# dongyunjinyu/YOLO-Lite

Hardware: NVIDIA B200
Metric: images_per_sec (higher is better)
Workload: dtype bf16

## Files before the change

include/yl11.h:

```cpp
#ifndef YL11_H
#define YL11_H

#include <stddef.h>
#include <stdint.h>

#ifdef __cplusplus
extern "C" {
#endif

#define YL11_VERSION 200

typedef enum yl_status {
    YL_OK = 0,
    YL_ERR_ARG = -1,
    YL_ERR_CUDA = -2,
    YL_ERR_UNSUPPORTED = -3,
    YL_ERR_WORKSPACE = -4,
    YL_ERR_NO_DEVICE = -5
} yl_status;

typedef enum yl_dtype { YL_BF16 = 0, YL_F32 = 1, YL_U8 = 2, YL_F16 = 3 } yl_dtype;
typedef enum yl_act { YL_ACT_NONE = 0, YL_ACT_SILU = 1 } yl_act;
typedef enum yl_conv_impl { YL_IMPL_AUTO = 0, YL_IMPL_DIRECT = 1, YL_IMPL_TCGEN05 = 2 } yl_conv_impl;

// ... 86 lines not shown
int yl_dw_pw_det_supported(const yl_conv_args* pw, const yl_conv_args* head);
int yl_dw_pw_det(const yl_conv_args* pw, const void* dw_w, const float* dw_bias, int dw_act, const yl_conv_args* head, void* stream);

int yl_sppf_pool(const yl_tensor* x, const yl_tensor* y1, const yl_tensor* y2, const yl_tensor* y3, int k,
                 void* stream);

int yl_psa_attention(const yl_tensor* qkv, const yl_tensor* out, int heads, int key_dim, int head_dim,
                     float scale, void* stream);

int yl_detect_decode(const yl_tensor* levels, int nl, const float* strides_host, int reg_max, int nc, float* y,
                     void* stream);

int yl_dfl(const float* x, float* y, int b, int reg_max, int a, void* stream);

size_t yl_nms_workspace_bytes(int B, int A, int nc, int multi_label);
int yl_nms_batched(const float* pred, int B, int nc, int A, float conf_thres, double iou_thres,
                   const int32_t* classes_dev, int n_classes, int agnostic, int multi_label, int max_det,
                   int max_nms, float max_wh, void* workspace, size_t workspace_bytes, float* out,
                   int32_t* counts, void* stream);
int yl_nms_begin(void* workspace, size_t workspace_bytes, int B, void* stream);
int yl_debug_nms_phases(long long* device_buf);
int yl_nms_select(const float* pred, int B, int nc, int A, double iou_thres, int agnostic, int max_det, int max_nms,
                  float max_wh, void* workspace, size_t workspace_bytes, float* out, int32_t* counts, void* stream);
size_t yl_nms_boxes_workspace_bytes(int n);
int yl_nms_boxes(const float* boxes, const float* scores, int n, double iou_thres, void* workspace,
                 size_t workspace_bytes, int64_t* keep, int32_t* count, void* stream);
int yl_xywh2xyxy_inplace(float* pred, int B, int C, int A, void* stream);
int yl_scale_boxes(float* dets, const int32_t* counts, int B, int max_det, const float* params_dev, void* stream);

int yl_to_f32(const void* x, int x_dtype, float* y, long long n, void* stream);

int yl_stem_fused_supported(int ci, int c0, int c1);
int yl_stem_fused(const void* x_nchw, int x_dtype, int n, int ci, int h, int w, const void* w0, int ci_pad0,
                  const float* b0, int act0, const void* w1, int ci_pad1, const float* b1, int act1, const yl_tensor* y,
                  void* stream);

int yl_c3k2_tail_supported(int c, int c2);
int yl_c3k2_tail(const yl_tensor* t, const yl_tensor* y, const void* wa, const float* ba, int wa_co_pad, int wa_ci_pad,
                 const void* wb, const float* bb, int wb_ci_pad, const void* w2, const float* b2, int w2_ci_pad,
                 int shortcut, void* stream);
int yl_c3k2_tail_tc(const yl_tensor* t, const yl_tensor* y, const void* wa, const float* ba, int wa_co_pad, int wa_ci_pad,
                 const void* wb, const float* bb, int wb_ci_pad, const void* w2, const float* b2, int w2_ci_pad,
                 int shortcut, void* stream);

int yl_match_predictions(const float* dets, const int32_t* counts, int B, int max_det, const float* gt_boxes,
                         const float* gt_cls, const int32_t* gt_offsets, int max_labels_per_image,
                         const float* iou_thresholds_dev, int n_thresholds, uint8_t* tp, void* stream);

typedef struct yl_lb_image {
    const uint8_t* src;
    int32_t sh, sw, pitch;
    int32_t new_w, new_h, left, top;
    int32_t _pad;
} yl_lb_image;
int yl_letterbox_u8(const yl_lb_image* imgs_dev, int n, float* dst_nchw, int H, int W, int pad_value, void* stream);

typedef struct yl_tta_canvas {
    float* y;
    int32_t H, W;
    int32_t h, w;
    int32_t flip;
    int32_t _pad;
} yl_tta_canvas;
int yl_tta_scale_img(const void* x, int x_dtype, int n, int c, int h, int w, const yl_tta_canvas* canvases, void* stream);
typedef struct yl_tta_pass {
    const float* pred;
    int32_t A;
    int32_t a0, n;
// ... 11 lines not shown
```

yolo-lite_b200/csrc/stem_fused.cu:

```cuda
#include <cuda_fp16.h>

#include "common.cuh"

namespace yl {

struct StemFusedParams {
    const void* x;
    int N, CI, H, W;
    const __nv_bfloat16* w0;
    int ci_pad0;
    const float* b0;
    const __nv_bfloat16* w1;
    const float* b1;
    __nv_bfloat16* y;
    long long y_cstride;
    int y_coff;
    int H0, W0, H1, W1;
    int act0, act1;
    int tiles_w, tiles_h, total_tiles;
};

__device__ __forceinline__ void sf_ldsm_x4(uint32_t addr, uint32_t& r0, uint32_t& r1, uint32_t& r2, uint32_t& r3) {
    asm volatile("ldmatrix.sync.aligned.m8n8.x4.shared.b16 {%0,%1,%2,%3}, [%4];"
                 : "=r"(r0), "=r"(r1), "=r"(r2), "=r"(r3)
                 : "r"(addr));
}
__device__ __forceinline__ void sf_mma(float (&d)[4], const uint32_t (&a)[4], uint32_t b0, uint32_t b1) {
    asm volatile(
        "mma.sync.aligned.m16n8k16.row.col.f32.bf16.bf16.f32 {%0,%1,%2,%3}, {%4,%5,%6,%7}, {%8,%9}, {%0,%1,%2,%3};"
        : "+f"(d[0]), "+f"(d[1]), "+f"(d[2]), "+f"(d[3])
        : "r"(a[0]), "r"(a[1]), "r"(a[2]), "r"(a[3]), "r"(b0), "r"(b1));
}

template <typename T> struct SfQuad;
template <> struct SfQuad<float> {
    using raw = float4;
    static __device__ __forceinline__ raw zero() { return make_float4(0.f, 0.f, 0.f, 0.f); }
    static __device__ __forceinline__ raw load(const float* p) { return __ldg(reinterpret_cast<const float4*>(p)); }
    static __device__ __forceinline__ float4 widen(raw v) { return v; }
    static __device__ __forceinline__ float one(const float* p) { return __ldg(p); }
};
template <> struct SfQuad<__half> {
    using raw = uint2;
    static __device__ __forceinline__ raw zero() { return make_uint2(0u, 0u); }
    static __device__ __forceinline__ raw load(const __half* p) { return __ldg(reinterpret_cast<const uint2*>(p)); }
    static __device__ __forceinline__ float4 widen(raw v) {
        const float2 a = __half22float2(*reinterpret_cast<const __half2*>(&v.x));
        const float2 b = __half22float2(*reinterpret_cast<const __half2*>(&v.y));
        return make_float4(a.x, a.y, b.x, b.y);
    }
    static __device__ __forceinline__ float one(const __half* p) { return __half2float(*p); }
};
template <> struct SfQuad<uint8_t> {
    using raw = uint32_t;
    static __device__ __forceinline__ raw zero() { return 0u; }
    static __device__ __forceinline__ raw load(const uint8_t* p) { return __ldg(reinterpret_cast<const uint32_t*>(p)); }
    static __device__ __forceinline__ float4 widen(raw v) {
        return make_float4(__fdiv_rn((float)(v & 0xffu), 255.f), __fdiv_rn((float)((v >> 8) & 0xffu), 255.f),
                           __fdiv_rn((float)((v >> 16) & 0xffu), 255.f), __fdiv_rn((float)(v >> 24), 255.f));
    }
    static __device__ __forceinline__ float one(const uint8_t* p) { return __fdiv_rn((float)__ldg(p), 255.f); }
};

constexpr int SF_TH = 8, SF_TW = 16;
constexpr int SF_R0 = 2 * SF_TH + 1, SF_C0 = 2 * SF_TW + 1;
constexpr int SF_RI = 2 * SF_R0 + 1;
constexpr int SF_CI = 72;
constexpr int SF_M0 = (SF_R0 * SF_C0 + 15) / 16;
constexpr int SF_EC = (SF_C0 + 1) / 2;
constexpr int SF_P0 = 48;
constexpr int SF_W1S = 9 * 16 * 2 + 16;
constexpr int SF_OFF_IN = 0;
constexpr int SF_OFF_L0 = SF_OFF_IN + SF_RI * SF_CI * 8;
constexpr int SF_OFF_W1 = SF_OFF_L0 + 2 * SF_R0 * SF_EC * SF_P0;
constexpr int SF_OFF_B = SF_OFF_W1 + 32 * SF_W1S;
constexpr int SF_OFF_TAB = SF_OFF_B + 48 * 4;
constexpr int SF_SMEM = SF_OFF_TAB + SF_M0 * 16 * 8;

template <typename TIn>
__global__ void __launch_bounds__(256, 2) stem_fused_kernel(const StemFusedParams p) {
    using Q = SfQuad<TIn>;
    const TIn* px_in = reinterpret_cast<const TIn*>(p.x);
    extern __shared__ __align__(16) uint8_t sf_smem[];
    griddep_launch_dependents();
    const int lane = threadIdx.x & 31, warp = threadIdx.x >> 5;
    const int g = lane >> 2, t = lane & 3;
    uint2* s_in = reinterpret_cast<uint2*>(sf_smem + SF_OFF_IN);
    const uint32_t sL0 = smem_u32(sf_smem + SF_OFF_L0), sW1 = smem_u32(sf_smem + SF_OFF_W1);
    float* sb0 = reinterpret_cast<float*>(sf_smem + SF_OFF_B);
    float* sb1 = sb0 + 16;

    for (int i = threadIdx.x; i < 32 * (SF_W1S / 16); i += blockDim.x) {
        const int r = i / (SF_W1S / 16), u = i - r * (SF_W1S / 16);
        uint4 v = make_uint4(0u, 0u, 0u, 0u);
        if (u < 18) v = __ldg(reinterpret_cast<const uint4*>(p.w1 + (size_t)r * 144) + u);
        *reinterpret_cast<uint4*>(sf_smem + SF_OFF_W1 + r * SF_W1S + u * 16) = v;
    }
    if (threadIdx.x < 16) sb0[threadIdx.x] = __ldg(p.b0 + threadIdx.x);
    if (threadIdx.x < 32) sb1[threadIdx.x] = __ldg(p.b1 + threadIdx.x);
    uint32_t bw0[3][2][2];
#pragma unroll
    for (int nt = 0; nt < 2; ++nt) {
        const __nv_bfloat16* wrow = p.w0 + (size_t)(nt * 8 + g) * 9 * p.ci_pad0;
#pragma unroll
        for (int ks = 0; ks < 3; ++ks)
#pragma unroll
            for (int hh = 0; hh < 2; ++hh) {
                uint32_t v = 0;
#pragma unroll
                for (int e = 0; e < 2; ++e) {
                    const int k = 16 * ks + 2 * t + e + hh * 8;
                    const int tap = k >> 2, ci = k & 3;
                    uint32_t bits = 0;
                    if (tap < 9 && ci < p.CI) bits = (uint32_t)__bfloat16_as_ushort(wrow[tap * p.ci_pad0 + ci]);
                    v |= bits << (16 * e);
                }
                bw0[ks][nt][hh] = v;
            }
    }
    int woff[3][2];
#pragma unroll
    for (int ks = 0; ks < 3; ++ks)
#pragma unroll
        for (int hh = 0; hh < 2; ++hh) {
            const int k = 16 * ks + 2 * t + hh * 8;
            const int tap = k >> 2, r = tap / 3, s2 = tap - 3 * r;
            woff[ks][hh] = tap < 9 ? ((r * SF_CI + s2) * 2 + ((k >> 1) & 1)) : 0;
        }
    uint2* s_tab = reinterpret_cast<uint2*>(sf_smem + SF_OFF_TAB);
    for (int i = threadIdx.x; i < SF_M0 * 16; i += blockDim.x) {
        const bool valid = i < SF_R0 * SF_C0;
        const int idx = valid ? i : SF_R0 * SF_C0 - 1;
// ... 133 lines not shown

        {
            const int r = warp;
            const int lrow = lane & 15, khalf = lane >> 4;
            float acc[4][4];
#pragma unroll
            for (int nt = 0; nt < 4; ++nt) {
                const float2 bb = *reinterpret_cast<const float2*>(sb1 + nt * 8 + 2 * t);
                acc[nt][0] = bb.x; acc[nt][1] = bb.y; acc[nt][2] = bb.x; acc[nt][3] = bb.y;
            }
            const uint32_t brow = sW1 + (uint32_t)(((lane >> 4) * 8 + (lane & 7)) * SF_W1S + 8 * ((lane >> 3) & 1) * 2);
#pragma unroll
            for (int t3 = 0; t3 < 9; t3 += 3) {
                uint32_t a[3][4], b[3][2][4];
#pragma unroll
                for (int j = 0; j < 3; ++j) {
                    const int tap = t3 + j, dr = tap / 3, dc = tap - 3 * dr;
                    const uint32_t arow = sL0 + (uint32_t)((((dc & 1) * SF_R0 + 2 * r + dr) * SF_EC + lrow + (dc >> 1)) * SF_P0 +
                                                           khalf * 16);
                    sf_ldsm_x4(arow, a[j][0], a[j][1], a[j][2], a[j][3]);
#pragma unroll
                    for (int np = 0; np < 2; ++np)
                        sf_ldsm_x4(brow + (uint32_t)(np * 16 * SF_W1S + tap * 32), b[j][np][0], b[j][np][1], b[j][np][2],
                                   b[j][np][3]);
                }
#pragma unroll
                for (int j = 0; j < 3; ++j)
#pragma unroll
                    for (int np = 0; np < 2; ++np) {
                        sf_mma(acc[2 * np], a[j], b[j][np][0], b[j][np][1]);
                        sf_mma(acc[2 * np + 1], a[j], b[j][np][2], b[j][np][3]);
                    }
            }
            const int oh = oh0 + r, ow = ow0 + g + 8 * (t >> 1);
            const bool st_ok = oh < p.H1 && ow < p.W1;
            __nv_bfloat16* yp = p.y + (((long long)n * p.H1 + oh) * p.W1 + ow) * p.y_cstride + p.y_coff + 8 * (t & 1);
#pragma unroll
            for (int np = 0; np < 2; ++np) {
                float e[2][4];
#pragma unroll
                for (int q = 0; q < 2; ++q)
#pragma unroll
                    for (int i = 0; i < 4; ++i) e[q][i] = p.act1 ? silu_fast(acc[2 * np + q][i]) : acc[2 * np + q][i];
                uint32_t v0 = pack_bf16x2(e[0][0], e[0][1]);
                uint32_t v1 = pack_bf16x2(e[1][0], e[1][1]);
                uint32_t v2 = pack_bf16x2(e[0][2], e[0][3]);
                uint32_t v3 = pack_bf16x2(e[1][2], e[1][3]);
                {
                    const uint32_t s0 = (t & 1) ? v0 : v1, s1 = (t & 1) ? v2 : v3;
                    const uint32_t r0 = __shfl_xor_sync(0xffffffffu, s0, 1), r1 = __shfl_xor_sync(0xffffffffu, s1, 1);
                    if (t & 1) { v0 = r0; v2 = r1; } else { v1 = r0; v3 = r1; }
                }
                {
                    const uint32_t s0 = (t & 2) ? v0 : v2, s1 = (t & 2) ? v1 : v3;
                    const uint32_t r0 = __shfl_xor_sync(0xffffffffu, s0, 2), r1 = __shfl_xor_sync(0xffffffffu, s1, 2);
                    if (t & 2) { v0 = r0; v1 = r1; } else { v2 = r0; v3 = r1; }
                }
                if (st_ok) *reinterpret_cast<uint4*>(yp + np * 16) = make_uint4(v0, v1, v2, v3);
            }
        }
        if (next < p.total_tiles) {
            if (vec_ok) patch_store();
            else patch_slow(next);
        }
        __syncthreads();
    }
}

static int g_sf_sms = 148;

int init_stem_fused() {
    int dev = 0;
    YL_CUDA(cudaGetDevice(&dev));
    YL_CUDA(cudaDeviceGetAttribute(&g_sf_sms, cudaDevAttrMultiProcessorCount, dev));
    YL_CUDA(cudaFuncSetAttribute(stem_fused_kernel<float>, cudaFuncAttributeMaxDynamicSharedMemorySize, SF_SMEM));
    YL_CUDA(cudaFuncSetAttribute(stem_fused_kernel<__half>, cudaFuncAttributeMaxDynamicSharedMemorySize, SF_SMEM));
    YL_CUDA(cudaFuncSetAttribute(stem_fused_kernel<uint8_t>, cudaFuncAttributeMaxDynamicSharedMemorySize, SF_SMEM));
    return YL_OK;
}

}

extern "C" int yl_stem_fused_supported(int ci, int c0, int c1) { return ci >= 1 && ci <= 3 && c0 == 16 && c1 == 32; }

extern "C" int yl_stem_fused(const void* x_nchw, int x_dtype, int n, int ci, int h, int w, const void* w0, int ci_pad0,
                             const float* b0, int act0, const void* w1, int ci_pad1, const float* b1, int act1,
                             const yl_tensor* y, void* stream) {
    YL_CHECK(x_nchw && w0 && b0 && w1 && b1 && y && y->data, YL_ERR_ARG, "null pointer");
    YL_CHECK(x_dtype == YL_F32 || x_dtype == YL_F16 || x_dtype == YL_U8, YL_ERR_ARG,
             "fused stem reads fp32, fp16 or uint8 images (got dtype %d)", x_dtype);
    YL_CHECK(y->dtype == YL_BF16, YL_ERR_ARG, "stem output must be bf16");
    YL_CHECK(yl_stem_fused_supported(ci, 16, y->c) && ci_pad1 == 16, YL_ERR_UNSUPPORTED,
             "fused stem is built for <= 3 input channels, 16 -> 32 (got ci = %d, c1 = %d, ci_pad1 = %d)", ci, y->c, ci_pad1);
    const int H0 = (h + 2 - 3) / 2 + 1, W0 = (w + 2 - 3) / 2 + 1;
    const int H1 = (H0 + 2 - 3) / 2 + 1, W1 = (W0 + 2 - 3) / 2 + 1;
    YL_CHECK(y->n == n && y->h == H1 && y->w == W1, YL_ERR_ARG, "fused stem output shape mismatch: got (%d,%d,%d) expected (%d,%d,%d)",
             y->n, y->h, y->w, n, H1, W1);
    YL_CHECK(y->coff % 8 == 0 && y->cstride % 8 == 0 && ((uintptr_t)y->data | (uintptr_t)w1) % 16 == 0, YL_ERR_ARG,
             "fused stem needs 8-channel / 16-byte alignment");
    YL_CHECK((long long)ci * h * w < (1ll << 31), YL_ERR_ARG, "image too large");
    yl::StemFusedParams p;
    p.x = x_nchw;
    p.N = n;
    p.CI = ci;
    p.H = h;
    p.W = w;
    p.w0 = reinterpret_cast<const __nv_bfloat16*>(w0);
    p.ci_pad0 = ci_pad0;
    p.b0 = b0;
    p.w1 = reinterpret_cast<const __nv_bfloat16*>(w1);
    p.b1 = b1;
    p.y = reinterpret_cast<__nv_bfloat16*>(y->data);
    p.y_cstride = y->cstride;
    p.y_coff = y->coff;
    p.H0 = H0;
    p.W0 = W0;
    p.H1 = H1;
    p.W1 = W1;
    p.act0 = act0;
    p.act1 = act1;
    p.tiles_w = yl::ceil_div(W1, yl::SF_TW);
    p.tiles_h = yl::ceil_div(H1, yl::SF_TH);
    p.total_tiles = p.tiles_w * p.tiles_h * n;
    const int sms = yl::g_sf_sms;
    int per_sm = (int)((size_t)220 * 1024 / (yl::SF_SMEM + 1024));
    per_sm = per_sm < 1 ? 1 : (per_sm > 2 ? 2 : per_sm);
    int grid = sms * per_sm;
    if (grid > p.total_tiles) grid = p.total_tiles;
    if (x_dtype == YL_F32)
        YL_CUDA(yl::launch_kernel(yl::stem_fused_kernel<float>, dim3(grid), dim3(256), (size_t)yl::SF_SMEM, (cudaStream_t)stream, p));
    else if (x_dtype == YL_F16)
        YL_CUDA(yl::launch_kernel(yl::stem_fused_kernel<__half>, dim3(grid), dim3(256), (size_t)yl::SF_SMEM, (cudaStream_t)stream, p));
    else
        YL_CUDA(yl::launch_kernel(yl::stem_fused_kernel<uint8_t>, dim3(grid), dim3(256), (size_t)yl::SF_SMEM, (cudaStream_t)stream, p));
    YL_LAUNCH_OK("stem_fused_kernel");
    return YL_OK;
}
```

yolo-lite_b200/yololite/_C.py:

```python
from __future__ import annotations

import ctypes as C
import os
from pathlib import Path

import torch

_LIB_PATH = Path(__file__).resolve().parent / "lib" / "libyl11.so"
_lib = None
_inited_devices: set[int] = set()

YL_BF16, YL_F32, YL_U8, YL_F16 = 0, 1, 2, 3
INGEST_DTYPES = {torch.float32: YL_F32, torch.float16: YL_F16, torch.uint8: YL_U8}
ACT_NONE, ACT_SILU = 0, 1
IMPL_AUTO, IMPL_DIRECT, IMPL_TCGEN05 = 0, 1, 2


class YLError(RuntimeError):
    """Raised for every non-zero yl_status."""


class Tensor(C.Structure):

    _fields_ = [
# ... 108 lines not shown
                                      C.c_void_p]),
    "yl_conv_chain_run": (C.c_int, [C.POINTER(ConvChain), C.c_void_p]),
    "yl_conv_chain_debug": (C.c_int, [C.c_void_p]),
    "yl_stem_conv": (C.c_int, [C.c_void_p, C.c_int, C.c_int, C.c_int, C.c_int, C.c_void_p, C.c_int, C.c_void_p,
                               C.POINTER(Tensor), C.c_int, C.c_void_p]),
    "yl_dwconv3x3": (C.c_int, [C.POINTER(Tensor), C.POINTER(Tensor), C.c_void_p, C.c_void_p, C.c_int,
                               C.POINTER(Tensor), C.c_void_p]),
    "yl_dw_pw_supported": (C.c_int, [C.POINTER(ConvArgs)]),
    "yl_dw_pw_conv": (C.c_int, [C.POINTER(ConvArgs), C.c_void_p, C.c_void_p, C.c_int, C.c_void_p]),
    "yl_dw_pw_det_supported": (C.c_int, [C.POINTER(ConvArgs), C.POINTER(ConvArgs)]),
    "yl_dw_pw_det": (C.c_int, [C.POINTER(ConvArgs), C.c_void_p, C.c_void_p, C.c_int, C.POINTER(ConvArgs), C.c_void_p]),
    "yl_sppf_pool": (C.c_int, [C.POINTER(Tensor)] * 4 + [C.c_int, C.c_void_p]),
    "yl_psa_attention": (C.c_int, [C.POINTER(Tensor), C.POINTER(Tensor), C.c_int, C.c_int, C.c_int, C.c_float,
                                   C.c_void_p]),
    "yl_detect_decode": (C.c_int, [C.POINTER(Tensor), C.c_int, C.POINTER(C.c_float), C.c_int, C.c_int, C.c_void_p,
                                   C.c_void_p]),
    "yl_dfl": (C.c_int, [C.c_void_p, C.c_void_p, C.c_int, C.c_int, C.c_int, C.c_void_p]),
    "yl_nms_workspace_bytes": (C.c_size_t, [C.c_int] * 4),
    "yl_nms_batched": (C.c_int, [C.c_void_p, C.c_int, C.c_int, C.c_int, C.c_float, C.c_double, C.c_void_p, C.c_int,
                                 C.c_int, C.c_int, C.c_int, C.c_int, C.c_float, C.c_void_p, C.c_size_t, C.c_void_p,
                                 C.c_void_p, C.c_void_p]),
    "yl_nms_begin": (C.c_int, [C.c_void_p, C.c_size_t, C.c_int, C.c_void_p]),
    "yl_debug_nms_phases": (C.c_int, [C.c_void_p]),
    "yl_nms_select": (C.c_int, [C.c_void_p, C.c_int, C.c_int, C.c_int, C.c_double, C.c_int, C.c_int, C.c_int, C.c_float,
                                C.c_void_p, C.c_size_t, C.c_void_p, C.c_void_p, C.c_void_p]),
    "yl_nms_boxes_workspace_bytes": (C.c_size_t, [C.c_int]),
    "yl_nms_boxes": (C.c_int, [C.c_void_p, C.c_void_p, C.c_int, C.c_double, C.c_void_p, C.c_size_t, C.c_void_p,
                               C.c_void_p, C.c_void_p]),
    "yl_xywh2xyxy_inplace": (C.c_int, [C.c_void_p, C.c_int, C.c_int, C.c_int, C.c_void_p]),
    "yl_scale_boxes": (C.c_int, [C.c_void_p, C.c_void_p, C.c_int, C.c_int, C.c_void_p, C.c_void_p]),
    "yl_to_f32": (C.c_int, [C.c_void_p, C.c_int, C.c_void_p, C.c_longlong, C.c_void_p]),
    "yl_stem_fused_supported": (C.c_int, [C.c_int, C.c_int, C.c_int]),
    "yl_stem_fused": (C.c_int, [C.c_void_p, C.c_int, C.c_int, C.c_int, C.c_int, C.c_int, C.c_void_p, C.c_int, C.c_void_p, C.c_int,
                                C.c_void_p, C.c_int, C.c_void_p, C.c_int, C.POINTER(Tensor), C.c_void_p]),
    "yl_c3k2_tail_supported": (C.c_int, [C.c_int, C.c_int]),
    "yl_c3k2_tail": (C.c_int, [C.POINTER(Tensor), C.POINTER(Tensor), C.c_void_p, C.c_void_p, C.c_int, C.c_int,
                               C.c_void_p, C.c_void_p, C.c_int, C.c_void_p, C.c_void_p, C.c_int, C.c_int, C.c_void_p]),
    "yl_c3k2_tail_tc": (C.c_int, [C.POINTER(Tensor), C.POINTER(Tensor), C.c_void_p, C.c_void_p, C.c_int, C.c_int,
                               C.c_void_p, C.c_void_p, C.c_int, C.c_void_p, C.c_void_p, C.c_int, C.c_int, C.c_void_p]),
    "yl_match_predictions": (C.c_int, [C.c_void_p, C.c_void_p, C.c_int, C.c_int, C.c_void_p, C.c_void_p, C.c_void_p, C.c_int,
                                       C.c_void_p, C.c_int, C.c_void_p, C.c_void_p]),
    "yl_letterbox_u8": (C.c_int, [C.c_void_p, C.c_int, C.c_void_p, C.c_int, C.c_int, C.c_int, C.c_void_p]),
    "yl_tta_scale_img": (C.c_int, [C.c_void_p, C.c_int, C.c_int, C.c_int, C.c_int, C.c_int, C.POINTER(TtaCanvas),
                                   C.c_void_p]),
    "yl_tta_merge": (C.c_int, [C.POINTER(TtaPass), C.c_int, C.c_int, C.c_int, C.c_void_p, C.c_void_p]),
}

EXPORTS = tuple(_PROTOTYPES)


def lib_path() -> Path:
    return _LIB_PATH


def load():
    global _lib
    if _lib is None:
        if not _LIB_PATH.exists():
            raise YLError(
                f"{_LIB_PATH} is missing: build it with `python yolo-lite_b200/csrc/build.py` "
                "(yololite has no CPU or library fallback)"
            )
        lib = C.CDLL(str(_LIB_PATH))
        for name, (res, args) in _PROTOTYPES.items():
            fn = getattr(lib, name)
            fn.restype = res
            fn.argtypes = args
# ... 52 lines not shown
```

yolo-lite_b200/yololite/_plan.py:

```python
from __future__ import annotations

import contextlib
import ctypes as C
import os
from typing import Callable

import torch

from . import _C, _ops
from ._ops import PackedConv, View


class Dest:

    def __init__(self, resolve: Callable[[int, int, int, int], View]):
        self._resolve = resolve

    def __call__(self, n, h, w, c) -> View:
        v = self._resolve(n, h, w, c)
        assert (v.n, v.h, v.w, v.c) == (n, h, w, c), f"destination {(v.n, v.h, v.w, v.c)} != {(n, h, w, c)}"
        return v


class DualDest:
# ... 196 lines not shown
        px = x.n * ho * wo
        rows = 4 if det.mode == _C.DET_BOX else det.nc
        self._push(self.lib.yl_conv_b2b_det, C.byref(a1), C.byref(a2), keep=(a1, a2, pc, plast, det), kind="conv_tc",
                   bytes_=px * x.c * 2 + px * rows * 4 + (pc.k * pc.k * x.c * pc.co + pc.co * plast.co) * 2,
                   flops=2 * px * (pc.k * pc.k * x.c * pc.co + pc.co * plast.co),
                   desc=f"[{x.c}->{pc.co} k{pc.k}s1, {pc.co}->{plast.co} k1 +decode] {x.h}x{x.w}", reads=(x,),
                   writes=((det.pred, 2 * det.anchor0 + (det.mode == _C.DET_CLS), 2 * det.anchor0 + (det.mode == _C.DET_CLS) + 1),))
        return True

    def dwpw_det(self, x: View, pdw: PackedConv, act_dw: bool, ppw: PackedConv, act_pw: bool, plast: PackedConv, det) -> bool:
        x = self.mat(x)
        if not (self.dwpw_enabled and self.dwpw_det_enabled and pdw.depthwise and pdw.k == 3 and ppw.k == 1 and plast.k == 1
                and not ppw.depthwise and not plast.depthwise and pdw.co == x.c and pdw.co_pad == x.c and ppw.ci == x.c
                and plast.ci == ppw.co):
            return False
        mid = _ops.NoOutput(x.n, x.h, x.w, ppw.co, torch.bfloat16)
        a1 = _ops.conv_args(x, mid, ppw, 1, act_pw, None, False, _C.IMPL_TCGEN05, None, None)
        a2 = _ops.conv_args(mid, _ops.NoOutput(x.n, x.h, x.w, plast.co, torch.float32), plast, 1, False, None, False,
                            _C.IMPL_TCGEN05, None, det)
        if not self.lib.yl_dw_pw_det_supported(C.byref(a1), C.byref(a2)):
            return False
        px = x.n * x.h * x.w
        filt = det.mode == _C.DET_CLS_FILTER
        self._push(self.lib.yl_dw_pw_det, C.byref(a1), pdw.w.data_ptr(), pdw.bias.data_ptr(), int(bool(act_dw)), C.byref(a2),
                   keep=(a1, a2, pdw, ppw, plast, det), kind="dwpw_tc",
                   bytes_=px * x.c * 2 + (0 if filt else px * det.nc * 4) + (9 * x.c + x.c * ppw.co + ppw.co * plast.co) * 2,
                   flops=2 * px * (9 * x.c + x.c * ppw.co + ppw.co * plast.co),
                   desc=f"[dw3x3 {x.c}, {x.c}->{ppw.co} k1, {ppw.co}->{plast.co} k1 {'+filter' if filt else '+decode'}] {x.h}x{x.w}",
                   reads=(x,),
                   writes=((det.cand_ws, 1 + det.anchor0, 2 + det.anchor0) if filt else
                           (det.pred, 2 * det.anchor0 + 1, 2 * det.anchor0 + 2),))
        return True

    def stem_fused(self, x: NchwInput, pc0: PackedConv, pc1: PackedConv, act0: bool, act1: bool, out=None) -> View:
        assert x.view is None and not self.calls, "the fused stem must be the first launch of the plan"
        h0, w0 = (x.h - 1) // 2 + 1, (x.w - 1) // 2 + 1
        h1, w1 = (h0 - 1) // 2 + 1, (w0 - 1) // 2 + 1
        y = self._out(out, x.n, h1, w1, pc1.co)
        yt = y.ct()
        self._push(self.lib.yl_stem_fused, x.static.data_ptr(), _C.YL_F32, x.n, x.c, x.h, x.w, pc0.w.data_ptr(), pc0.ci_pad,
                   pc0.bias.data_ptr(), int(act0), pc1.w.data_ptr(), pc1.ci_pad, pc1.bias.data_ptr(), int(act1),
                   C.byref(yt), keep=(yt, pc0, pc1, x.static), kind="stem_fused",
                   bytes_=x.n * x.c * x.h * x.w * 4 + x.n * h1 * w1 * pc1.co * 2,
                   flops=2 * x.n * (h0 * w0 * pc0.co * x.c * 9 + h1 * w1 * pc1.co * pc0.co * 9),
                   desc=f"[{x.c}->{pc0.co} k3s2, {pc0.co}->{pc1.co} k3s2] {x.h}x{x.w} nchw-f32 in", writes=(y,))
        return y

    def c3k2_tail(self, t: View, pa: PackedConv, pb: PackedConv, p2: PackedConv, shortcut: bool, out=None,
                  impl: str = "auto") -> View:
        y = self._out(out, t.n, t.h, t.w, p2.co)
        tt, yt = t.ct(), y.ct()
        c = t.c // 2
        px = t.n * t.h * t.w
        self._push(self.lib.yl_c3k2_tail_tc if impl == "tc" else self.lib.yl_c3k2_tail, C.byref(tt), C.byref(yt),
                   pa.w.data_ptr(), pa.bias.data_ptr(), pa.co_pad,
                   pa.ci_pad, pb.w.data_ptr(), pb.bias.data_ptr(), pb.ci_pad, p2.w.data_ptr(), p2.bias.data_ptr(),
                   p2.ci_pad, int(bool(shortcut)), keep=(tt, yt, pa, pb, p2), kind="c3k2_tail",
                   bytes_=px * (t.c + p2.co) * 2 + (pa.w.numel() + pb.w.numel() + p2.w.numel()) * 2,
                   flops=2 * px * (9 * c * (c // 2) * 2 + 3 * c * p2.co),
                   desc=f"[{c}->{c // 2} k3, {c // 2}->{c} k3{' +res' if shortcut else ''}, {3 * c}->{p2.co} k1] "
                        f"{t.h}x{t.w}", reads=(t,), writes=(y,))
        return y

    def sppf_pool(self, x: View, y1: View, y2: View, y3: View, k: int):
        ts = [v.ct() for v in (x, y1, y2, y3)]
        self._push(self.lib.yl_sppf_pool, *[C.byref(t) for t in ts], k, keep=tuple(ts), kind="sppf_pool",
                   bytes_=x.n * x.h * x.w * x.c * 2 * 4, reads=(x,), writes=(y1, y2, y3))

    def upsample2x(self, x: View, out=None) -> View:
        x = self.mat(x)
        y = self._out(out, x.n, 2 * x.h, 2 * x.w, x.c)
        xt, yt = x.ct(), y.ct()
        self._push(self.lib.yl_upsample2x, C.byref(xt), C.byref(yt), keep=(xt, yt), kind="upsample2x",
                   bytes_=x.n * x.h * x.w * x.c * 2 * 5, reads=(x,), writes=(y,))
        return y

    def copy(self, x: View, out=None) -> View:
        x = self.mat(x)
# ... 273 lines not shown
```

yolo-lite_b200/yololite/nn/modules/block.py:

```python
from __future__ import annotations

import torch
import torch.nn as nn

from ._emit import YLModule, emit_any, packed
from .conv import Conv

__all__ = ("DFL", "SPPF", "C2f", "C3", "C3k", "C3k2", "Bottleneck", "Attention", "PSABlock", "C2PSA")


class DFL(YLModule):

    def __init__(self, c1=16):
        super().__init__()
        self.conv = nn.Conv2d(c1, 1, 1, bias=False).requires_grad_(False)
        self.conv.weight.data[:] = torch.arange(c1, dtype=torch.float).view(1, c1, 1, 1)
        self.c1 = c1

    def forward(self, x):
        from ... import _ops

        if not x.is_cuda:
            raise RuntimeError("yololite modules run on CUDA (sm_100) only")
        return _ops.dfl_expectation(x, self.c1)
# ... 19 lines not shown
        self.c = int(c2 * e)
        self.cv1 = Conv(c1, 2 * self.c, 1, 1)
        self.cv2 = Conv((2 + n) * self.c, c2, 1)
        self.m = nn.ModuleList(Bottleneck(self.c, self.c, shortcut, g, k=((3, 3), (3, 3)), e=1.0) for _ in range(n))

    fuse_tail = True
    fuse_tail_max_c = 16
    tail_impl = "auto"

    def _tail_fusable(self, out):
        import os

        from ... import _C, _plan
        from ._emit import act_flag

        if not self.fuse_tail or os.environ.get("YL_C3K2_FUSE", "1") == "0" or len(self.m) != 1:
            return False
        b = self.m[0]
        if type(b) is not Bottleneck or isinstance(out, _plan.DualDest):
            return False
        convs = (b.cv1, b.cv2, self.cv2)
        if any(type(cv) is not Conv or not hasattr(cv, "bn") or not act_flag(cv.act) or cv.conv.groups != 1
               or cv.conv.stride != (1, 1) for cv in convs):
            return False
        if b.cv1.conv.kernel_size != (3, 3) or b.cv2.conv.kernel_size != (3, 3) or self.cv2.conv.kernel_size != (1, 1):
            return False
        c = self.c
        if c > self.fuse_tail_max_c:
            return False
        if b.cv1.conv.in_channels != c or b.cv1.conv.out_channels != c // 2 or b.cv2.conv.out_channels != c:
            return False
        return bool(_C.load().yl_c3k2_tail_supported(c, self.cv2.conv.out_channels))

    def _emit(self, g, x, out=None):
        c, n = self.c, len(self.m)
        if self._tail_fusable(out):
            t = self.cv1._emit(g, x)
            b = self.m[0]
            return g.c3k2_tail(t, packed(b.cv1.conv, b.cv1.bn, b.cv1), packed(b.cv2.conv, b.cv2.bn, b.cv2),
                               packed(self.cv2.conv, self.cv2.bn, self.cv2), b.add, out=out, impl=self.tail_impl)
        cat = g.alloc(x.n, x.h, x.w, (2 + n) * c)
        self.cv1._emit(g, x, out=cat.slice(0, 2 * c))
        prev = cat.slice(c, c)
        for i, m in enumerate(self.m):
            prev = m._emit(g, prev, out=cat.slice((2 + i) * c, c))
        return self.cv2._emit(g, cat, out=out)

    forward_split = YLModule.forward


class C3(YLModule):

    def __init__(self, c1, c2, n=1, shortcut=True, g=1, e=0.5):
        super().__init__()
        c_ = int(c2 * e)
        self.cv1 = Conv(c1, c_, 1, 1)
        self.cv2 = Conv(c1, c_, 1, 1)
        self.cv3 = Conv(2 * c_, c2, 1)
        self.m = nn.Sequential(*(Bottleneck(c_, c_, shortcut, g, k=((1, 1), (3, 3)), e=1.0) for _ in range(n)))

    def _merged_pack(self):
        from ... import _ops

        a, b = self.cv1, self.cv2
        ca, cb = a.conv, b.conv
        same = (ca.kernel_size == cb.kernel_size == (1, 1) and ca.stride == cb.stride == (1, 1)
                and ca.groups == cb.groups == 1 and ca.in_channels == cb.in_channels
                and ca.out_channels == cb.out_channels and ca.out_channels % 8 == 0 and ca.bias is None
                and cb.bias is None and type(a.act) is type(b.act) and hasattr(a, "bn") and hasattr(b, "bn")
                and a.bn.eps == b.bn.eps)
        if not same:
            return None
        pc = self.__dict__.get("_yl_pc12")
        dev = ca.weight.device
        if pc is None or pc.w.device != dev:
# ... 141 lines not shown
```

yolo-lite_b200/yololite/nn/tasks.py:

```python
from __future__ import annotations

import ast
import math
import re
from copy import deepcopy
from pathlib import Path
from typing import NamedTuple

import torch
import torch.nn as nn

from .. import _plan
from ..cfg import CFG_DIR, DEFAULT_CFG_DICT
from ..utils import LOGGER, yaml_load
from .modules import (C2PSA, C3, SPPF, Bottleneck, C2f, C3k, C3k2, Concat, Conv, Detect, DWConv)
from .modules._emit import YLModule, emit_any

_MODULES = {m.__name__: m for m in (Conv, DWConv, Bottleneck, SPPF, C2f, C3, C3k, C3k2, C2PSA, Concat, Detect)}
_REPEATABLE = {C2f, C3, C3k2, C2PSA}
_CHANNEL_ARGS = {Conv, DWConv, Bottleneck, SPPF, C2f, C3, C3k2, C2PSA}


def make_divisible(x, divisor):
    if isinstance(divisor, torch.Tensor):
# ... 158 lines not shown
        if visualize or embed or profile:
            raise NotImplementedError("visualize / embed / profile are not part of the inference hot path")
        if augment and self._augment_supported():
            y, _ = self.infer(x, augment=True)
            return (y.clone() if self.clone_outputs else y), None
        out = self.infer(x, want_raw=True)
        if self.clone_outputs:
            y, raws = out
            return y.clone(), [r.clone() for r in raws]
        return out

    _predict_once = predict

    def _layer_scales(self):
        sc = []
        for m in self.model:
            f = m.f
            src = (sc[f] if f != -1 else (sc[-1] if sc else 1.0)) if isinstance(f, int) else \
                [(sc[j] if j != -1 else sc[-1]) for j in f]
            if isinstance(m, Conv):
                s = src * m.conv.stride[0]
            elif isinstance(m, nn.Upsample):
                s = src / float(m.scale_factor)
            elif isinstance(m, Concat):
                s = src[0]
            elif isinstance(m, Detect):
                s = src
            else:
                s = src
            sc.append(s)
        return sc

    def _emit(self, g, x, out=None):
        from .._ops import View

        layers = list(self.model)
        n_layers = len(layers)
        srcs = []
        for i, m in enumerate(layers):
            f = [m.f] if isinstance(m.f, int) else list(m.f)
            srcs.append([(i - 1 if j == -1 else (j if j >= 0 else i + j)) for j in f])
        n_cat_uses = [0] * n_layers
        for i, m in enumerate(layers):
            if isinstance(m, Concat):
                for j in srcs[i]:
                    if j >= 0:
                        n_cat_uses[j] += 1
        place, cat_buf = {}, {}
        for i, m in enumerate(layers):
            if isinstance(m, Concat) and all(j >= 0 and n_cat_uses[j] == 1 for j in srcs[i]) \
                    and len(set(srcs[i])) == len(srcs[i]):
                for j in srcs[i]:
                    place[j] = i
        ys: list = [None] * n_layers
        out_ch = {}

        def dest_for(j):
            ci = place.get(j)
            if ci is None:
                return None

            def resolve(n, h, w, c, j=j, ci=ci):
                if ci not in cat_buf:
                    chans = [self._out_channels(layers, k, out_ch) for k in srcs[ci]]
                    cat_buf[ci] = (g.alloc(n, h, w, sum(chans)), chans)
                buf, chans = cat_buf[ci]
                off = sum(chans[: srcs[ci].index(j)])
                return buf.slice(off, c)

            return _plan.Dest(resolve)

        n_uses = [0] * n_layers
        for i in range(n_layers):
            for j in srcs[i]:
                if j >= 0:
                    n_uses[j] += 1
        fused_up = {}
        for u, m in enumerate(layers):
            if isinstance(m, nn.Upsample) and m.mode == "nearest" and float(m.scale_factor) == 2.0:
                j = srcs[u][0]
                if j >= 0 and isinstance(layers[j], (Conv, C2f, C3, SPPF, C2PSA)) and j not in fused_up:
                    fused_up[j] = u
        done_up = {}

        fuse_stem = self._stem_fusable(g, x, layers, srcs, n_uses)
        cur = x
        for i, m in enumerate(layers):
            if fuse_stem and i == 0:
                continue
            if fuse_stem and i == 1:
                from .modules._emit import act_flag, packed

                l0, l1 = layers[0], layers[1]
                cur = ys[1] = g.stem_fused(x, packed(l0.conv, l0.bn, l0), packed(l1.conv, l1.bn, l1), act_flag(l0.act),
                                           act_flag(l1.act), out=dest_for(1))
                continue
            inp = [ys[j] if j >= 0 else x for j in srcs[i]]
            if isinstance(m, Detect):
                return m._emit(g, inp)
            if isinstance(m, Concat):
                if i in cat_buf and all(place.get(j) == i for j in srcs[i]):
                    buf, chans = cat_buf[i]
                    cur = View(buf.buf, buf.coff, sum(chans))
                else:
                    cur = m._emit(g, inp, out=dest_for(i))
            elif i in done_up:
                cur = done_up[i]
            elif i in fused_up:
                u = fused_up[i]
                dd = _plan.DualDest(dest_for(i), dest_for(u))
                cur = emit_any(g, m, inp[0], out=dd)
                assert dd.up_view is not None, f"layer {i}: producer did not honour the fused upsample"
                done_up[u] = dd.up_view
            else:
                cur = emit_any(g, m, inp[0], out=dest_for(i))
            ys[i] = cur
        return cur

    fuse_stem = True

    def _stem_fusable(self, g, x, layers, srcs, n_uses):
        import os

        from .. import _C

        if not self.fuse_stem or os.environ.get("YL_STEM_FUSE", "1") == "0" or len(layers) < 3:
            return False
        if not isinstance(x, _plan.NchwInput) or x.view is not None or g.calls:
            return False
        l0, l1 = layers[0], layers[1]
        if type(l0) is not Conv or type(l1) is not Conv or srcs[1] != [0] or n_uses[0] != 1 or 1 in fused_up_guard(layers):
            return False
        for cv in (l0, l1):
            c = cv.conv
            if c.kernel_size != (3, 3) or c.stride != (2, 2) or c.groups != 1 or not hasattr(cv, "bn") or c.bias is not None:
                return False
        if l0.conv.in_channels != x.c:
            return False
        return bool(_C.load().yl_stem_fused_supported(x.c, l0.conv.out_channels, l1.conv.out_channels))

    @staticmethod
    def _out_channels(layers, k, memo):
        if k in memo:
            return memo[k]
        m = layers[k]
        if isinstance(m, Conv):
            c = m.conv.out_channels
        elif isinstance(m, (C2f, SPPF, C2PSA, C3)):
            c = m.cv2.conv.out_channels if not isinstance(m, C3) else m.cv3.conv.out_channels
        elif isinstance(m, Concat):
            f = [m.f] if isinstance(m.f, int) else list(m.f)
            c = sum(BaseModel._out_channels(layers, (k - 1 if j == -1 else j), memo) for j in f)
        elif isinstance(m, nn.Sequential):
            c = BaseModel._out_channels(list(m), len(m) - 1, {})
        else:
            j = m.f if isinstance(m.f, int) else m.f[0]
            c = BaseModel._out_channels(layers, k - 1 if j == -1 else j, memo)
        memo[k] = c
        return c

    def _get_plan(self, shape, dev, want_raw=False, slot=0, nms=None):
        plans = self.__dict__.setdefault("_yl_plans", {})
        key = (tuple(shape), dev.index, bool(self.use_cuda_graph), bool(want_raw), int(slot), nms)
        entry = plans.get(key)
        if entry is not None:
            plans[key] = plans.pop(key)
        else:
            if len(plans) >= max(int(self.max_plans), 1):
                torch.cuda.synchronize(dev)
                plans.pop(next(iter(plans)))
            with torch.cuda.device(dev):
                g = _plan.Builder(dev)
# ... 191 lines not shown
```

Before: 41000.

## Fuse first C2f cv1 1x1 conv into the fused stem kernel

Extends the fused stem kernel with an optional third 1x1 32->32 conv, computed from the layer-1 accumulators held in registers through an extra MMA stage with weights staged in shared memory. The planner routes the first C2f block's cv1 through the stem, so the intermediate layer-1 activation is never written to or read back from global memory and one launch disappears. It also raises the launch bound and the per-SM block cap from 2 to 3, which could force register spills given the extra accumulator work.

```diff
diff --git a/include/yl11.h b/include/yl11.h
--- a/include/yl11.h
+++ b/include/yl11.h
@@ -142,8 +142,8 @@
 
 int yl_stem_fused_supported(int ci, int c0, int c1);
 int yl_stem_fused(const void* x_nchw, int x_dtype, int n, int ci, int h, int w, const void* w0, int ci_pad0,
-                  const float* b0, int act0, const void* w1, int ci_pad1, const float* b1, int act1, const yl_tensor* y,
-                  void* stream);
+                  const float* b0, int act0, const void* w1, int ci_pad1, const float* b1, int act1, const void* w2,
+                  int ci_pad2, const float* b2, int act2, const yl_tensor* y, void* stream);
 
 int yl_c3k2_tail_supported(int c, int c2);
 int yl_c3k2_tail(const yl_tensor* t, const yl_tensor* y, const void* wa, const float* ba, int wa_co_pad, int wa_ci_pad,
diff --git a/yolo-lite_b200/csrc/stem_fused.cu b/yolo-lite_b200/csrc/stem_fused.cu
--- a/yolo-lite_b200/csrc/stem_fused.cu
+++ b/yolo-lite_b200/csrc/stem_fused.cu
@@ -12,11 +12,13 @@
     const float* b0;
     const __nv_bfloat16* w1;
     const float* b1;
+    const __nv_bfloat16* w2;
+    const float* b2;
     __nv_bfloat16* y;
     long long y_cstride;
     int y_coff;
     int H0, W0, H1, W1;
-    int act0, act1;
+    int act0, act1, act2;
     int tiles_w, tiles_h, total_tiles;
 };
 
@@ -73,12 +75,14 @@
 constexpr int SF_OFF_IN = 0;
 constexpr int SF_OFF_L0 = SF_OFF_IN + SF_RI * SF_CI * 8;
 constexpr int SF_OFF_W1 = SF_OFF_L0 + 2 * SF_R0 * SF_EC * SF_P0;
-constexpr int SF_OFF_B = SF_OFF_W1 + 32 * SF_W1S;
-constexpr int SF_OFF_TAB = SF_OFF_B + 48 * 4;
+constexpr int SF_W2S = 32 * 2 + 16;
+constexpr int SF_OFF_W2 = SF_OFF_W1 + 32 * SF_W1S;
+constexpr int SF_OFF_B = SF_OFF_W2 + 32 * SF_W2S;
+constexpr int SF_OFF_TAB = SF_OFF_B + 80 * 4;
 constexpr int SF_SMEM = SF_OFF_TAB + SF_M0 * 16 * 8;
 
 template <typename TIn>
-__global__ void __launch_bounds__(256, 2) stem_fused_kernel(const StemFusedParams p) {
+__global__ void __launch_bounds__(256, 3) stem_fused_kernel(const StemFusedParams p) {
     using Q = SfQuad<TIn>;
     const TIn* px_in = reinterpret_cast<const TIn*>(p.x);
     extern __shared__ __align__(16) uint8_t sf_smem[];
@@ -87,8 +91,11 @@
     const int g = lane >> 2, t = lane & 3;
     uint2* s_in = reinterpret_cast<uint2*>(sf_smem + SF_OFF_IN);
     const uint32_t sL0 = smem_u32(sf_smem + SF_OFF_L0), sW1 = smem_u32(sf_smem + SF_OFF_W1);
+    const uint32_t sW2 = smem_u32(sf_smem + SF_OFF_W2);
     float* sb0 = reinterpret_cast<float*>(sf_smem + SF_OFF_B);
     float* sb1 = sb0 + 16;
+    float* sb2 = sb0 + 48;
+    const bool has2 = p.w2 != nullptr;
 
     for (int i = threadIdx.x; i < 32 * (SF_W1S / 16); i += blockDim.x) {
         const int r = i / (SF_W1S / 16), u = i - r * (SF_W1S / 16);
@@ -96,8 +103,15 @@
         if (u < 18) v = __ldg(reinterpret_cast<const uint4*>(p.w1 + (size_t)r * 144) + u);
         *reinterpret_cast<uint4*>(sf_smem + SF_OFF_W1 + r * SF_W1S + u * 16) = v;
     }
+    if (has2 && threadIdx.x < 32 * (SF_W2S / 16)) {
+        const int r = threadIdx.x / (SF_W2S / 16), u = threadIdx.x - r * (SF_W2S / 16);
+        uint4 v = make_uint4(0u, 0u, 0u, 0u);
+        if (u < 4) v = __ldg(reinterpret_cast<const uint4*>(p.w2 + (size_t)r * 32) + u);
+        *reinterpret_cast<uint4*>(sf_smem + SF_OFF_W2 + r * SF_W2S + u * 16) = v;
+    }
     if (threadIdx.x < 16) sb0[threadIdx.x] = __ldg(p.b0 + threadIdx.x);
     if (threadIdx.x < 32) sb1[threadIdx.x] = __ldg(p.b1 + threadIdx.x);
+    if (has2 && threadIdx.x < 32) sb2[threadIdx.x] = __ldg(p.b2 + threadIdx.x);
     uint32_t bw0[3][2][2];
 #pragma unroll
     for (int nt = 0; nt < 2; ++nt) {
@@ -297,6 +311,40 @@
                         sf_mma(acc[2 * np + 1], a[j], b[j][np][2], b[j][np][3]);
                     }
             }
+            int act_out = p.act1;
+            if (has2) {
+                uint32_t a2[2][4];
+#pragma unroll
+                for (int ks = 0; ks < 2; ++ks)
+#pragma unroll
+                    for (int q = 0; q < 2; ++q) {
+                        float e[4];
+#pragma unroll
+                        for (int i = 0; i < 4; ++i) e[i] = p.act1 ? silu_fast(acc[2 * ks + q][i]) : acc[2 * ks + q][i];
+                        a2[ks][2 * q] = pack_bf16x2(e[0], e[1]);
+                        a2[ks][2 * q + 1] = pack_bf16x2(e[2], e[3]);
+                    }
+#pragma unroll
+                for (int nt = 0; nt < 4; ++nt)
+#pragma unroll
+                    for (int i = 0; i < 4; ++i) acc[nt][i] = 0.f;
+                const uint32_t brow2 = sW2 + (uint32_t)(((lane >> 4) * 8 + (lane & 7)) * SF_W2S + 16 * ((lane >> 3) & 1));
+#pragma unroll
+                for (int ks = 0; ks < 2; ++ks)
+#pragma unroll
+                    for (int np = 0; np < 2; ++np) {
+                        uint32_t b[4];
+                        sf_ldsm_x4(brow2 + (uint32_t)(np * 16 * SF_W2S + ks * 32), b[0], b[1], b[2], b[3]);
+                        sf_mma(acc[2 * np], a2[ks], b[0], b[1]);
+                        sf_mma(acc[2 * np + 1], a2[ks], b[2], b[3]);
+                    }
+#pragma unroll
+                for (int nt = 0; nt < 4; ++nt) {
+                    const float2 bb = *reinterpret_cast<const float2*>(sb2 + nt * 8 + 2 * t);
+                    acc[nt][0] += bb.x; acc[nt][1] += bb.y; acc[nt][2] += bb.x; acc[nt][3] += bb.y;
+                }
+                act_out = p.act2;
+            }
             const int oh = oh0 + r, ow = ow0 + g + 8 * (t >> 1);
             const bool st_ok = oh < p.H1 && ow < p.W1;
             __nv_bfloat16* yp = p.y + (((long long)n * p.H1 + oh) * p.W1 + ow) * p.y_cstride + p.y_coff + 8 * (t & 1);
@@ -306,7 +354,7 @@
 #pragma unroll
                 for (int q = 0; q < 2; ++q)
 #pragma unroll
-                    for (int i = 0; i < 4; ++i) e[q][i] = p.act1 ? silu_fast(acc[2 * np + q][i]) : acc[2 * np + q][i];
+                    for (int i = 0; i < 4; ++i) e[q][i] = act_out ? silu_fast(acc[2 * np + q][i]) : acc[2 * np + q][i];
                 uint32_t v0 = pack_bf16x2(e[0][0], e[0][1]);
                 uint32_t v1 = pack_bf16x2(e[1][0], e[1][1]);
                 uint32_t v2 = pack_bf16x2(e[0][2], e[0][3]);
@@ -350,8 +398,10 @@
 
 extern "C" int yl_stem_fused(const void* x_nchw, int x_dtype, int n, int ci, int h, int w, const void* w0, int ci_pad0,
                              const float* b0, int act0, const void* w1, int ci_pad1, const float* b1, int act1,
-                             const yl_tensor* y, void* stream) {
+                             const void* w2, int ci_pad2, const float* b2, int act2, const yl_tensor* y, void* stream) {
     YL_CHECK(x_nchw && w0 && b0 && w1 && b1 && y && y->data, YL_ERR_ARG, "null pointer");
+    YL_CHECK(!w2 || (b2 && ci_pad2 == 32 && (uintptr_t)w2 % 16 == 0), YL_ERR_UNSUPPORTED,
+             "fused stem's third conv must be a 1x1 32 -> 32 with 16-byte aligned weights (got ci_pad2 = %d)", ci_pad2);
     YL_CHECK(x_dtype == YL_F32 || x_dtype == YL_F16 || x_dtype == YL_U8, YL_ERR_ARG,
              "fused stem reads fp32, fp16 or uint8 images (got dtype %d)", x_dtype);
     YL_CHECK(y->dtype == YL_BF16, YL_ERR_ARG, "stem output must be bf16");
@@ -375,6 +425,8 @@
     p.b0 = b0;
     p.w1 = reinterpret_cast<const __nv_bfloat16*>(w1);
     p.b1 = b1;
+    p.w2 = reinterpret_cast<const __nv_bfloat16*>(w2);
+    p.b2 = b2;
     p.y = reinterpret_cast<__nv_bfloat16*>(y->data);
     p.y_cstride = y->cstride;
     p.y_coff = y->coff;
@@ -384,12 +436,13 @@
     p.W1 = W1;
     p.act0 = act0;
     p.act1 = act1;
+    p.act2 = act2;
     p.tiles_w = yl::ceil_div(W1, yl::SF_TW);
     p.tiles_h = yl::ceil_div(H1, yl::SF_TH);
     p.total_tiles = p.tiles_w * p.tiles_h * n;
     const int sms = yl::g_sf_sms;
     int per_sm = (int)((size_t)220 * 1024 / (yl::SF_SMEM + 1024));
-    per_sm = per_sm < 1 ? 1 : (per_sm > 2 ? 2 : per_sm);
+    per_sm = per_sm < 1 ? 1 : (per_sm > 3 ? 3 : per_sm);
     int grid = sms * per_sm;
     if (grid > p.total_tiles) grid = p.total_tiles;
     if (x_dtype == YL_F32)
diff --git a/yolo-lite_b200/yololite/_C.py b/yolo-lite_b200/yololite/_C.py
--- a/yolo-lite_b200/yololite/_C.py
+++ b/yolo-lite_b200/yololite/_C.py
@@ -164,7 +164,8 @@
     "yl_to_f32": (C.c_int, [C.c_void_p, C.c_int, C.c_void_p, C.c_longlong, C.c_void_p]),
     "yl_stem_fused_supported": (C.c_int, [C.c_int, C.c_int, C.c_int]),
     "yl_stem_fused": (C.c_int, [C.c_void_p, C.c_int, C.c_int, C.c_int, C.c_int, C.c_int, C.c_void_p, C.c_int, C.c_void_p, C.c_int,
-                                C.c_void_p, C.c_int, C.c_void_p, C.c_int, C.POINTER(Tensor), C.c_void_p]),
+                                C.c_void_p, C.c_int, C.c_void_p, C.c_int, C.c_void_p, C.c_int, C.c_void_p, C.c_int,
+                                C.POINTER(Tensor), C.c_void_p]),
     "yl_c3k2_tail_supported": (C.c_int, [C.c_int, C.c_int]),
     "yl_c3k2_tail": (C.c_int, [C.POINTER(Tensor), C.POINTER(Tensor), C.c_void_p, C.c_void_p, C.c_int, C.c_int,
                                C.c_void_p, C.c_void_p, C.c_int, C.c_void_p, C.c_void_p, C.c_int, C.c_int, C.c_void_p]),
diff --git a/yolo-lite_b200/yololite/_plan.py b/yolo-lite_b200/yololite/_plan.py
--- a/yolo-lite_b200/yololite/_plan.py
+++ b/yolo-lite_b200/yololite/_plan.py
@@ -252,18 +252,23 @@
                            (det.pred, 2 * det.anchor0 + 1, 2 * det.anchor0 + 2),))
         return True
 
-    def stem_fused(self, x: NchwInput, pc0: PackedConv, pc1: PackedConv, act0: bool, act1: bool, out=None) -> View:
+    def stem_fused(self, x: NchwInput, pc0: PackedConv, pc1: PackedConv, act0: bool, act1: bool, out=None,
+                   pc2: PackedConv | None = None, act2: bool = False) -> View:
         assert x.view is None and not self.calls, "the fused stem must be the first launch of the plan"
         h0, w0 = (x.h - 1) // 2 + 1, (x.w - 1) // 2 + 1
         h1, w1 = (h0 - 1) // 2 + 1, (w0 - 1) // 2 + 1
-        y = self._out(out, x.n, h1, w1, pc1.co)
+        co = pc2.co if pc2 is not None else pc1.co
+        y = self._out(out, x.n, h1, w1, co)
         yt = y.ct()
+        third = (pc2.w.data_ptr(), pc2.ci_pad, pc2.bias.data_ptr(), int(act2)) if pc2 is not None else (None, 0, None, 0)
         self._push(self.lib.yl_stem_fused, x.static.data_ptr(), _C.YL_F32, x.n, x.c, x.h, x.w, pc0.w.data_ptr(), pc0.ci_pad,
-                   pc0.bias.data_ptr(), int(act0), pc1.w.data_ptr(), pc1.ci_pad, pc1.bias.data_ptr(), int(act1),
-                   C.byref(yt), keep=(yt, pc0, pc1, x.static), kind="stem_fused",
-                   bytes_=x.n * x.c * x.h * x.w * 4 + x.n * h1 * w1 * pc1.co * 2,
-                   flops=2 * x.n * (h0 * w0 * pc0.co * x.c * 9 + h1 * w1 * pc1.co * pc0.co * 9),
-                   desc=f"[{x.c}->{pc0.co} k3s2, {pc0.co}->{pc1.co} k3s2] {x.h}x{x.w} nchw-f32 in", writes=(y,))
+                   pc0.bias.data_ptr(), int(act0), pc1.w.data_ptr(), pc1.ci_pad, pc1.bias.data_ptr(), int(act1), *third,
+                   C.byref(yt), keep=(yt, pc0, pc1, pc2, x.static), kind="stem_fused",
+                   bytes_=x.n * x.c * x.h * x.w * 4 + x.n * h1 * w1 * co * 2,
+                   flops=2 * x.n * (h0 * w0 * pc0.co * x.c * 9 + h1 * w1 * pc1.co * pc0.co * 9
+                                    + (h1 * w1 * co * pc1.co if pc2 is not None else 0)),
+                   desc=f"[{x.c}->{pc0.co} k3s2, {pc0.co}->{pc1.co} k3s2"
+                        f"{f', {pc1.co}->{co} k1' if pc2 is not None else ''}] {x.h}x{x.w} nchw-f32 in", writes=(y,))
         return y
 
     def c3k2_tail(self, t: View, pa: PackedConv, pb: PackedConv, p2: PackedConv, shortcut: bool, out=None,
diff --git a/yolo-lite_b200/yololite/nn/modules/block.py b/yolo-lite_b200/yololite/nn/modules/block.py
--- a/yolo-lite_b200/yololite/nn/modules/block.py
+++ b/yolo-lite_b200/yololite/nn/modules/block.py
@@ -75,15 +75,17 @@
             return False
         return bool(_C.load().yl_c3k2_tail_supported(c, self.cv2.conv.out_channels))
 
-    def _emit(self, g, x, out=None):
+    def _emit(self, g, x, out=None, cv1=None):
         c, n = self.c, len(self.m)
+        if cv1 is None:
+            cv1 = lambda dest: self.cv1._emit(g, x, out=dest)
         if self._tail_fusable(out):
-            t = self.cv1._emit(g, x)
+            t = cv1(None)
             b = self.m[0]
             return g.c3k2_tail(t, packed(b.cv1.conv, b.cv1.bn, b.cv1), packed(b.cv2.conv, b.cv2.bn, b.cv2),
                                packed(self.cv2.conv, self.cv2.bn, self.cv2), b.add, out=out, impl=self.tail_impl)
         cat = g.alloc(x.n, x.h, x.w, (2 + n) * c)
-        self.cv1._emit(g, x, out=cat.slice(0, 2 * c))
+        cv1(cat.slice(0, 2 * c))
         prev = cat.slice(c, c)
         for i, m in enumerate(self.m):
             prev = m._emit(g, prev, out=cat.slice((2 + i) * c, c))
diff --git a/yolo-lite_b200/yololite/nn/tasks.py b/yolo-lite_b200/yololite/nn/tasks.py
--- a/yolo-lite_b200/yololite/nn/tasks.py
+++ b/yolo-lite_b200/yololite/nn/tasks.py
@@ -214,7 +214,7 @@
         return sc
 
     def _emit(self, g, x, out=None):
-        from .._ops import View
+        from .._ops import NoOutput, View
 
         layers = list(self.model)
         n_layers = len(layers)
@@ -266,6 +266,7 @@
         done_up = {}
 
         fuse_stem = self._stem_fusable(g, x, layers, srcs, n_uses)
+        stem_cv1 = fuse_stem and self._stem_takes_cv1(layers, srcs, n_uses)
         cur = x
         for i, m in enumerate(layers):
             if fuse_stem and i == 0:
@@ -274,8 +275,18 @@
                 from .modules._emit import act_flag, packed
 
                 l0, l1 = layers[0], layers[1]
-                cur = ys[1] = g.stem_fused(x, packed(l0.conv, l0.bn, l0), packed(l1.conv, l1.bn, l1), act_flag(l0.act),
-                                           act_flag(l1.act), out=dest_for(1))
+
+                def stem(dest, cv=None, l0=l0, l1=l1):
+                    return g.stem_fused(x, packed(l0.conv, l0.bn, l0), packed(l1.conv, l1.bn, l1), act_flag(l0.act),
+                                        act_flag(l1.act), out=dest, pc2=None if cv is None else packed(cv.conv, cv.bn, cv),
+                                        act2=cv is not None and act_flag(cv.act))
+                if not stem_cv1:
+                    cur = ys[1] = stem(dest_for(1))
+                continue
+            if stem_cv1 and i == 2:
+                h0, w0 = (x.h - 1) // 2 + 1, (x.w - 1) // 2 + 1
+                shape = NoOutput(x.n, (h0 - 1) // 2 + 1, (w0 - 1) // 2 + 1, layers[1].conv.out_channels, torch.bfloat16)
+                cur = ys[2] = m._emit(g, shape, out=dest_for(2), cv1=lambda dest, cv=m.cv1: stem(dest, cv))
                 continue
             inp = [ys[j] if j >= 0 else x for j in srcs[i]]
             if isinstance(m, Detect):
@@ -320,6 +331,17 @@
         if l0.conv.in_channels != x.c:
             return False
         return bool(_C.load().yl_stem_fused_supported(x.c, l0.conv.out_channels, l1.conv.out_channels))
+
+    @staticmethod
+    def _stem_takes_cv1(layers, srcs, n_uses):
+        m = layers[2]
+        if not isinstance(m, C2f) or srcs[2] != [1] or n_uses[1] != 1 or 2 in fused_up_guard(layers):
+            return False
+        cv = m.cv1
+        c = cv.conv
+        return (type(cv) is Conv and hasattr(cv, "bn") and c.bias is None and c.kernel_size == (1, 1)
+                and c.stride == (1, 1) and c.groups == 1 and c.in_channels == layers[1].conv.out_channels == 32
+                and c.out_channels == 32)
 
     @staticmethod
     def _out_channels(layers, k, memo):
```

Result: no change. 41100, median of 6 (+0.2%).
